# usmandroid/80211ParallelEstimation

Hardware: AMD Instinct MI355X
Metric: MMSE-estimated 802.11 frames/sec (53 subcarriers) at 1/2/4/8 MI355X; % roofline (higher is better)
Workload: dtype f64; 1 GPU; PS_MMSE textbook, BASELINE configs[2]; frames_per_gpu=65536, global_frames=65536, subcarriers=53, ofdm_blocks=15, parallelism=dp1 (frames sharded, 1 RCCL state broadcast)

## Files before the change

80211parallelestimation_amd/csrc/wce_rank1.hip:

```cpp
#include "wce_internal.h"
#include "wce_device.h"

namespace wce {

__device__ __forceinline__ double2 r1_mul(double2 a, double2 b)
{
#pragma clang fp contract(off)
    return make_double2(a.x * b.x - a.y * b.y, a.x * b.y + a.y * b.x);
}
__device__ __forceinline__ double2 r1_add(double2 a, double2 b)
{
#pragma clang fp contract(off)
    return make_double2(a.x + b.x, a.y + b.y);
}

__device__ __forceinline__ double2 rank1_p(double2 u, double2 w, bool cwg)
{
#pragma clang fp contract(off)
    return cwg ? r1_mul(w, u) : make_double2(u.x * u.x + u.y * u.y, 0.0);
}

__device__ __forceinline__ double2 rank1_s(const double2 (&x)[4], const double2 (&r)[4], const double2 (&u)[4],
                                           const double2 (&w)[4], const double2 (&p)[4], bool cwg, double ac,
                                           double bc)
{
#pragma clang fp contract(off)
    double2 g = make_double2(0.0, 0.0), q = g;
#pragma unroll
    for (int m = 0; m < 4; ++m) {
        const double ax2 = ac * (x[m].x * x[m].x + x[m].y * x[m].y);
        const double2 gk = make_double2(ax2 * p[m].x, ax2 * p[m].y);
        const double2 qk = r1_mul(r1_mul(w[m], cconj(x[m])), r[m]);
        g = m ? r1_add(g, gk) : gk;
        q = m ? r1_add(q, qk) : qk;
    }
    g = row16_sum(g);
    q = row16_sum(q);
    const double2 d = make_double2(bc + g.x, g.y);
    double2 t;
    if (cwg) {
        const double den = d.x * d.x + d.y * d.y;
        t = make_double2((q.x * d.x + q.y * d.y) / den, (q.y * d.x - q.x * d.y) / den);
    } else {
        t = make_double2(q.x / d.x, q.y / d.x);
    }
    double2 c = make_double2(0.0, 0.0);
#pragma unroll
    for (int m = 0; m < 4; ++m) {
        const double2 xu = r1_mul(x[m], u[m]);
        const double2 at = r1_mul(make_double2(ac * xu.x, ac * xu.y), t);
        const double2 rho = make_double2(r[m].x - at.x, r[m].y - at.y);
        const double ti = 2.0 * x[m].y;
        const double2 ck = r1_mul(w[m], make_double2(-(ti * rho.y), ti * rho.x));
        c = m ? r1_add(c, ck) : ck;
    }
    c = row16_sum(c);
    return make_double2(t.x + c.x / bc, t.y + c.y / bc);
}

constexpr int R1_WG_PER_CU = 4;
constexpr int R1_POL_DEFAULT = 0, R1_POL_NT = 1, R1_POL_NT_STORES = 2, R1_POL_NT_LOADS = 3;

constexpr bool r1_prefetch(bool noise, bool shared) { return shared && !noise; }

template <int POL, bool NOISE, bool SHARED, bool SPLIT, bool PF>
__global__ __launch_bounds__(256, R1_WG_PER_CU) void mmse_rank1_kernel(const State *__restrict__ st, SolveArgs a)
{
    static_assert(!PF || r1_prefetch(NOISE, SHARED), "this instantiation has no registers for a second unit");
    constexpr bool NTL = POL == R1_POL_NT || POL == R1_POL_NT_LOADS;
    constexpr bool NTS = POL == R1_POL_NT || POL == R1_POL_NT_STORES;
    const int i = threadIdx.x & 15;
    const uint32_t units = (uint32_t)(SPLIT ? a.n * a.nblk : a.n);
    const uint32_t rows = gridDim.x * 16u;
    uint32_t g = blockIdx.x * 16u + (threadIdx.x >> 4);
    if (g >= units) return;
    const bool cwg = !SHARED && a.cw != nullptr;
    const double ac = st->acoef;
    const uint64_t xm = st->xmask;
    const double2 zero = make_double2(0.0, 0.0);
    auto lane_again = [](int l) __attribute__((always_inline)) {
        asm volatile("" : "+v"(l));
        return l;
    };
    auto frame_of = [&](uint32_t gu) __attribute__((always_inline)) { return SPLIT ? gu / (uint32_t)a.nblk : gu; };
    auto fetch = [&](uint32_t gu, double2(&xl)[4], double2(&rl)[4], double &bc) __attribute__((always_inline)) {
        const uint32_t f = frame_of(gu);
        const int b = SPLIT ? (int)(gu - f * (uint32_t)a.nblk) : 0;
        const int64_t base = (int64_t)f * a.fs + (int64_t)(a.blk + b) * a.bs + lane_again(i);
#pragma unroll
        for (int m = 0; m < 3; ++m) {
            xl[m] = NTL ? ld2_nt(a.tx, base + 16 * m) : ld2(a.tx, base + 16 * m);
            rl[m] = NTL ? ld2_nt(a.rx, base + 16 * m) : ld2(a.rx, base + 16 * m);
        }
        xl[3] = zero;
        rl[3] = zero;
        if (i < NSC - 48) {
            xl[3] = NTL ? ld2_nt(a.tx, base + 48) : ld2(a.tx, base + 48);
            rl[3] = NTL ? ld2_nt(a.rx, base + 48) : ld2(a.rx, base + 48);
        }
        if (NOISE) bc = a.ow2[f];
    };
    auto factors = [&](int64_t cb, double2(&u)[4], double2(&w)[4], double2(&p)[4]) __attribute__((always_inline)) {
        const int64_t ub = cb + i;
#pragma unroll
        for (int m = 0; m < 3; ++m) {
            u[m] = ld2(a.cu, ub + 16 * m);
            w[m] = cwg ? ld2(a.cw, ub + 16 * m) : cconj(u[m]);
        }
        u[3] = zero;
        w[3] = zero;
        if (i < NSC - 48) {
            u[3] = ld2(a.cu, ub + 48);
            w[3] = cwg ? ld2(a.cw, ub + 48) : cconj(u[3]);
        }
#pragma unroll
        for (int m = 0; m < 4; ++m) p[m] = rank1_p(u[m], w[m], cwg);
    };
    double2 u[4], w[4], p[4];
    if (SHARED) factors(0, u, w, p);
    auto trip = [&](double2(&xc)[4], double2(&rc)[4], double &bc, double2(&xn)[4], double2(&rn)[4], double &bn)
                    __attribute__((always_inline)) {
        if (!PF) fetch(g, xc, rc, bc);
        const uint32_t f = frame_of(g);
        if (!SHARED) factors((int64_t)f * a.cs, u, w, p);
        const bool more = g + rows < units;
        if (PF && more) fetch(g + rows, xn, rn, bn);
        double2 x[4];
#pragma unroll
        for (int m = 0; m < 4; ++m)
            x[m] = (xm >> ((i + 16 * m) & 63)) & 1ull ? xc[m] : zero;
        double2 pl[4];
#pragma unroll
        for (int m = 0; m < 4; ++m) {
            double2 um = u[m];
            if (PF) asm volatile("" : "+v"(um.x), "+v"(um.y));
            pl[m] = PF ? rank1_p(um, w[m], cwg) : p[m];
        }
        double2 s = rank1_s(x, rc, u, w, pl, cwg, ac, bc);
        if (NOISE && !(bc > 0.0 && bc < __builtin_inf())) s = make_double2(__builtin_nan(""), __builtin_nan(""));
        if (SPLIT) {
            if (i == 0) st2(a.dots, g, s);
        } else {
            const int64_t hb = (int64_t)f * a.ws + lane_again(i);
#pragma unroll
            for (int m = 0; m < 4; ++m) {
                if (i + 16 * m < NSC) {
                    const double2 h = r1_mul(u[m], s);
                    if (NTS) st2_nt(a.w, hb + 16 * m, h);
                    else st2(a.w, hb + 16 * m, h);
                }
            }
        }
        g += rows;
        return more;
    };
    double2 xc[4], rc[4], xn[4], rn[4];
    double bc = st->bcoef, bn = bc;
    if (!PF) {
        while (trip(xc, rc, bc, xn, rn, bn)) {}
        return;
    }
    fetch(g, xc, rc, bc);
    bool more = trip(xc, rc, bc, xn, rn, bn);
    while (more) {
        bc = bn;
#pragma unroll
        for (int m = 0; m < 4; ++m) {
            xc[m] = xn[m];
            rc[m] = rn[m];
        }
        more = trip(xc, rc, bc, xn, rn, bn);
    }
}

int rank1_rows_per_sweep(int cus) { return (cus > 0 ? cus : 256) * R1_WG_PER_CU * 16; }

template <int POL, bool NOISE, bool SHARED>
static void launch_r1_split(const State *st, const SolveArgs &a, bool pf, dim3 g, hipStream_t s)
{
    const dim3 b(256);
    if constexpr (r1_prefetch(NOISE, SHARED)) {
        if (pf) {
            if (a.split) hipLaunchKernelGGL((mmse_rank1_kernel<POL, NOISE, SHARED, true, true>), g, b, 0, s, st, a);
            else hipLaunchKernelGGL((mmse_rank1_kernel<POL, NOISE, SHARED, false, true>), g, b, 0, s, st, a);
            return;
        }
    }
    if (a.split) hipLaunchKernelGGL((mmse_rank1_kernel<POL, NOISE, SHARED, true, false>), g, b, 0, s, st, a);
    else hipLaunchKernelGGL((mmse_rank1_kernel<POL, NOISE, SHARED, false, false>), g, b, 0, s, st, a);
}
template <int POL>
static void launch_r1_pol(const State *st, const SolveArgs &a, bool pf, dim3 g, hipStream_t s)
{
    const bool shared = a.cs == 0 && !a.cw;
    if (a.ow2) {
        if (shared) launch_r1_split<POL, true, true>(st, a, pf, g, s);
        else launch_r1_split<POL, true, false>(st, a, pf, g, s);
    } else {
        if (shared) launch_r1_split<POL, false, true>(st, a, pf, g, s);
        else launch_r1_split<POL, false, false>(st, a, pf, g, s);
    }
}

int launch_mmse_rank1(const State *st, const SolveArgs &a, bool nt, int cus, void *stream)
{
    if (!a.cu) return WCE_EINVAL;
    if (a.split ? !a.dots : !a.w) return WCE_EINVAL;
    if (a.n <= 0) return WCE_OK;
    if (a.nblk > 1 && !a.split) return WCE_EINVAL;
    if (a.ow2 && a.cw) return WCE_EINVAL;
    const int64_t units = a.split ? a.n * a.nblk : a.n;
    if (units > 0x7fffffffll) return WCE_EINVAL;
    const int shape = variant_value(WCE_VARIANT_R1);
    int64_t wgs = (units + 15) / 16;
    const bool looping = shape == 4 || shape == 7;
    const int64_t cap = shape == 4 ? 3 : shape == 7 ? rank1_rows_per_sweep(cus) / 16 : wgs;
    if (wgs > cap) wgs = cap;
    const dim3 g((unsigned)wgs);
    hipStream_t s = (hipStream_t)stream;
    if (nt) launch_r1_pol<R1_POL_NT>(st, a, looping, g, s);
    else if (shape == 5) launch_r1_pol<R1_POL_NT_STORES>(st, a, looping, g, s);
    else if (shape == 6) launch_r1_pol<R1_POL_NT_LOADS>(st, a, looping, g, s);
    else launch_r1_pol<R1_POL_DEFAULT>(st, a, looping, g, s);
    return hipGetLastError() == hipSuccess ? WCE_OK : WCE_EHIP;
}

}
```

Measured before the change: 2.213 billion frames/s.

## Issue rank-1 frame loads before factor loads and add smaller workgroup shapes

```diff
diff --git a/80211parallelestimation_amd/csrc/wce_rank1.hip b/80211parallelestimation_amd/csrc/wce_rank1.hip
--- a/80211parallelestimation_amd/csrc/wce_rank1.hip
+++ b/80211parallelestimation_amd/csrc/wce_rank1.hip
@@ -60,6 +60,7 @@
 
 constexpr int R1_WG_PER_CU = 4;
 constexpr int R1_POL_DEFAULT = 0, R1_POL_NT = 1, R1_POL_NT_STORES = 2, R1_POL_NT_LOADS = 3;
+constexpr int R1_POL_U_FIRST = 4;
 
 constexpr bool r1_prefetch(bool noise, bool shared) { return shared && !noise; }
 
@@ -69,14 +70,31 @@
     static_assert(!PF || r1_prefetch(NOISE, SHARED), "this instantiation has no registers for a second unit");
     constexpr bool NTL = POL == R1_POL_NT || POL == R1_POL_NT_LOADS;
     constexpr bool NTS = POL == R1_POL_NT || POL == R1_POL_NT_STORES;
+    constexpr bool LF = POL != R1_POL_U_FIRST;
     const int i = threadIdx.x & 15;
-    const uint32_t units = (uint32_t)(SPLIT ? a.n * a.nblk : a.n);
-    const uint32_t rows = gridDim.x * 16u;
-    uint32_t g = blockIdx.x * 16u + (threadIdx.x >> 4);
+    const uint32_t rpw = blockDim.x >> 4;
+    int64_t n = a.n;
+    if (LF) {
+        auto held = [](int64_t &c, auto v) __attribute__((always_inline)) { asm("" : "+s"(c) : "s"(v)); };
+        held(n, st), held(n, a.tx), held(n, a.rx), held(n, a.fs), held(n, a.bs), held(n, a.blk), held(n, a.cu);
+        held(n, rpw), held(n, gridDim.x);
+        if (SPLIT) held(n, a.nblk), held(n, a.dots);
+        else held(n, a.w), held(n, a.ws);
+        if (NOISE) held(n, a.ow2);
+        if (!SHARED) held(n, a.cs), held(n, a.cw);
+    }
+    const uint32_t units = (uint32_t)(SPLIT ? n * a.nblk : n);
+    const uint32_t rows = gridDim.x * rpw;
+    uint32_t g = blockIdx.x * rpw + (threadIdx.x >> 4);
     if (g >= units) return;
     const bool cwg = !SHARED && a.cw != nullptr;
-    const double ac = st->acoef;
-    const uint64_t xm = st->xmask;
+    double ac;
+    uint64_t xm;
+    auto scalars = [&](double &b) __attribute__((always_inline)) {
+        ac = st->acoef;
+        xm = st->xmask;
+        if (!NOISE) b = st->bcoef;
+    };
     const double2 zero = make_double2(0.0, 0.0);
     auto lane_again = [](int l) __attribute__((always_inline)) {
         asm volatile("" : "+v"(l));
@@ -102,25 +120,48 @@
     };
     auto factors = [&](int64_t cb, double2(&u)[4], double2(&w)[4], double2(&p)[4]) __attribute__((always_inline)) {
         const int64_t ub = cb + i;
-#pragma unroll
-        for (int m = 0; m < 3; ++m) {
-            u[m] = ld2(a.cu, ub + 16 * m);
-            w[m] = cwg ? ld2(a.cw, ub + 16 * m) : cconj(u[m]);
-        }
-        u[3] = zero;
-        w[3] = zero;
-        if (i < NSC - 48) {
-            u[3] = ld2(a.cu, ub + 48);
-            w[3] = cwg ? ld2(a.cw, ub + 48) : cconj(u[3]);
+        const bool live = i < NSC - 48;
+        if (SHARED) {
+#pragma unroll
+            for (int m = 0; m < 3; ++m) {
+                u[m] = ld2(a.cu, ub + 16 * m);
+                w[m] = cconj(u[m]);
+            }
+            u[3] = zero;
+            w[3] = zero;
+            if (live) {
+                u[3] = ld2(a.cu, ub + 48);
+                w[3] = cconj(u[3]);
+            }
+        } else {
+#pragma unroll
+            for (int m = 0; m < 3; ++m) u[m] = ld2(a.cu, ub + 16 * m);
+            u[3] = zero;
+            if (live) u[3] = ld2(a.cu, ub + 48);
+            if (cwg) {
+#pragma unroll
+                for (int m = 0; m < 3; ++m) w[m] = ld2(a.cw, ub + 16 * m);
+                w[3] = zero;
+                if (live) w[3] = ld2(a.cw, ub + 48);
+            } else {
+#pragma unroll
+                for (int m = 0; m < 3; ++m) w[m] = cconj(u[m]);
+                w[3] = live ? cconj(u[3]) : zero;
+            }
         }
 #pragma unroll
         for (int m = 0; m < 4; ++m) p[m] = rank1_p(u[m], w[m], cwg);
     };
     double2 u[4], w[4], p[4];
+    double2 xc[4], rc[4], xn[4], rn[4];
+    double bc = 0.0, bn;
+    scalars(bc);
+    if (LF) fetch(g, xc, rc, bc);
     if (SHARED) factors(0, u, w, p);
+    bn = bc;
     auto trip = [&](double2(&xc)[4], double2(&rc)[4], double &bc, double2(&xn)[4], double2(&rn)[4], double &bn)
                     __attribute__((always_inline)) {
-        if (!PF) fetch(g, xc, rc, bc);
+        if (!PF && !LF) fetch(g, xc, rc, bc);
         const uint32_t f = frame_of(g);
         if (!SHARED) factors((int64_t)f * a.cs, u, w, p);
         const bool more = g + rows < units;
@@ -154,13 +195,12 @@
         g += rows;
         return more;
     };
-    double2 xc[4], rc[4], xn[4], rn[4];
-    double bc = st->bcoef, bn = bc;
     if (!PF) {
-        while (trip(xc, rc, bc, xn, rn, bn)) {}
+        while (trip(xc, rc, bc, xn, rn, bn))
+            if (LF) fetch(g, xc, rc, bc);
         return;
     }
-    fetch(g, xc, rc, bc);
+    if (!LF) fetch(g, xc, rc, bc);
     bool more = trip(xc, rc, bc, xn, rn, bn);
     while (more) {
         bc = bn;
@@ -175,30 +215,34 @@
 
 int rank1_rows_per_sweep(int cus) { return (cus > 0 ? cus : 256) * R1_WG_PER_CU * 16; }
 
+struct R1Shape {
+    dim3 g, b;
+    bool pf;
+};
+
 template <int POL, bool NOISE, bool SHARED>
-static void launch_r1_split(const State *st, const SolveArgs &a, bool pf, dim3 g, hipStream_t s)
-{
-    const dim3 b(256);
+static void launch_r1_split(const State *st, const SolveArgs &a, const R1Shape &h, hipStream_t s)
+{
     if constexpr (r1_prefetch(NOISE, SHARED)) {
-        if (pf) {
-            if (a.split) hipLaunchKernelGGL((mmse_rank1_kernel<POL, NOISE, SHARED, true, true>), g, b, 0, s, st, a);
-            else hipLaunchKernelGGL((mmse_rank1_kernel<POL, NOISE, SHARED, false, true>), g, b, 0, s, st, a);
+        if (h.pf) {
+            if (a.split) hipLaunchKernelGGL((mmse_rank1_kernel<POL, NOISE, SHARED, true, true>), h.g, h.b, 0, s, st, a);
+            else hipLaunchKernelGGL((mmse_rank1_kernel<POL, NOISE, SHARED, false, true>), h.g, h.b, 0, s, st, a);
             return;
         }
     }
-    if (a.split) hipLaunchKernelGGL((mmse_rank1_kernel<POL, NOISE, SHARED, true, false>), g, b, 0, s, st, a);
-    else hipLaunchKernelGGL((mmse_rank1_kernel<POL, NOISE, SHARED, false, false>), g, b, 0, s, st, a);
+    if (a.split) hipLaunchKernelGGL((mmse_rank1_kernel<POL, NOISE, SHARED, true, false>), h.g, h.b, 0, s, st, a);
+    else hipLaunchKernelGGL((mmse_rank1_kernel<POL, NOISE, SHARED, false, false>), h.g, h.b, 0, s, st, a);
 }
 template <int POL>
-static void launch_r1_pol(const State *st, const SolveArgs &a, bool pf, dim3 g, hipStream_t s)
+static void launch_r1_pol(const State *st, const SolveArgs &a, const R1Shape &h, hipStream_t s)
 {
     const bool shared = a.cs == 0 && !a.cw;
     if (a.ow2) {
-        if (shared) launch_r1_split<POL, true, true>(st, a, pf, g, s);
-        else launch_r1_split<POL, true, false>(st, a, pf, g, s);
+        if (shared) launch_r1_split<POL, true, true>(st, a, h, s);
+        else launch_r1_split<POL, true, false>(st, a, h, s);
     } else {
-        if (shared) launch_r1_split<POL, false, true>(st, a, pf, g, s);
-        else launch_r1_split<POL, false, false>(st, a, pf, g, s);
+        if (shared) launch_r1_split<POL, false, true>(st, a, h, s);
+        else launch_r1_split<POL, false, false>(st, a, h, s);
     }
 }
 
@@ -212,16 +256,18 @@
     const int64_t units = a.split ? a.n * a.nblk : a.n;
     if (units > 0x7fffffffll) return WCE_EINVAL;
     const int shape = variant_value(WCE_VARIANT_R1);
-    int64_t wgs = (units + 15) / 16;
+    const int rpw = shape == 8 ? 4 : shape == 9 ? 8 : 16;
+    int64_t wgs = (units + rpw - 1) / rpw;
     const bool looping = shape == 4 || shape == 7;
     const int64_t cap = shape == 4 ? 3 : shape == 7 ? rank1_rows_per_sweep(cus) / 16 : wgs;
     if (wgs > cap) wgs = cap;
-    const dim3 g((unsigned)wgs);
+    const R1Shape h{dim3((unsigned)wgs), dim3(16u * rpw), looping};
     hipStream_t s = (hipStream_t)stream;
-    if (nt) launch_r1_pol<R1_POL_NT>(st, a, looping, g, s);
-    else if (shape == 5) launch_r1_pol<R1_POL_NT_STORES>(st, a, looping, g, s);
-    else if (shape == 6) launch_r1_pol<R1_POL_NT_LOADS>(st, a, looping, g, s);
-    else launch_r1_pol<R1_POL_DEFAULT>(st, a, looping, g, s);
+    if (nt) launch_r1_pol<R1_POL_NT>(st, a, h, s);
+    else if (shape == 5) launch_r1_pol<R1_POL_NT_STORES>(st, a, h, s);
+    else if (shape == 6) launch_r1_pol<R1_POL_NT_LOADS>(st, a, h, s);
+    else if (shape == 10) launch_r1_pol<R1_POL_U_FIRST>(st, a, h, s);
+    else launch_r1_pol<R1_POL_DEFAULT>(st, a, h, s);
     return hipGetLastError() == hipSuccess ? WCE_OK : WCE_EHIP;
 }
 
```

After: 2.255 billion frames/s, median of 6. 1.9% higher.
